# winddori2002/DEX-TTS

Hardware: AMD Instinct MI355X
Metric: mel-frames/s at n_timesteps=50, 80-ch mel (sampler only); RTF (higher is better)
Workload: dtype bf16; 1 GPU; gedex_b1: gedex_lj B=1/GPU T=512 n_timesteps=50 (BASELINE.json configs[1]); global_batch=1, frames=512, hipgraph=False, parallelism=1 GPU

## Files before the change

### dex_tts_amd/csrc/conv3x3_bf16.hip

```cpp
#include "kernels.h"
#include <cstdlib>
#include <cstdio>
#include "lp_util.h"
#include "kernels_lp.h"
#include "conv_gn.h"

namespace dex {
namespace DEX_LP_NS {

typedef float f32x16 __attribute__((ext_vector_type(16)));
typedef unsigned short u16;
typedef unsigned u32x4 __attribute__((ext_vector_type(4)));

__device__ __forceinline__ float cv_mish(float x) {
    const float e = __expf(fminf(x, 20.f));
    const float n = e * (e + 2.f);
    return x * (n * __builtin_amdgcn_rcpf(n + 2.f));
}

template <int NT, int COUT>
__device__ __forceinline__ void cv_epilogue(const Conv3P& p, f32x16 (&acc)[NT], int b, int ho, int w0, int nbase, int lane, int tid,
                                            long long* gnred) {
    const int i = lane & 31, hh = lane >> 5;
    constexpr int cpg = COUT / 8;
// ... 76 lines not shown
    const bool odd = (lane & 1) != 0;
#pragma unroll
    for (int t = 0; t < NT; ++t) {
        const float bias = p.res_b[nb + t * 32 + i];
        if (rfull) {
            float* yp = yl + (odd ? 16 * COUT - 1 : 0) + t * 32;
#pragma unroll
            for (int j = 0; j < 8; ++j) {
                const float lo_r = accr[t][j] + bias, hi_r = accr[t][8 + j] + bias;
                const float recv = lane_xor1(odd ? lo_r : hi_r);
                const float mine = odd ? hi_r : lo_r;
                *reinterpret_cast<float2*>(yp + ((j & 3) + 8 * (j >> 2)) * COUT) = odd ? make_float2(recv, mine) : make_float2(mine, recv);
            }
        } else {
#pragma unroll
            for (int r = 0; r < 16; ++r) {
                const int wo = w0 + (r & 3) + 8 * (r >> 2) + 4 * hh;
                if (ho < p.H && wo < p.W) yl[((r & 3) + 8 * (r >> 2)) * COUT + t * 32] = accr[t][r] + bias;
            }
        }
    }
}

template <int CC, int COUT, int NSL, int TH, bool PRO2 = false, bool RES = false, bool XB = false, int NW = 4, bool RW = false>
__global__ __launch_bounds__(64 * NW) void conv3x3_lp_kernel(const Conv3P p) {
    constexpr int PW = 34, PH = TH + 2;
    constexpr int LDP = CC + 8;
    constexpr int WN = NW / TH;
    constexpr int NTHR = 64 * NW;
    constexpr int NT = NSL / 32 / WN;
    constexpr int NSLICE = COUT / NSL;
    constexpr int ITEMS = PH * PW * (CC / 8);
    constexpr int NI = (ITEMS + NTHR - 1) / NTHR;
    constexpr int WITEMS = NSL * CC / 8;
    constexpr int WPT = (WITEMS + NTHR - 1) / NTHR;
    constexpr bool WFULL = WITEMS % NTHR == 0;
    constexpr int RING = CC == 128 ? (PRO2 ? 1 : 2) : 3;
    constexpr int NPASS = RW ? 1
                        : TH == 5 ? (CC == 128 ? (PRO2 ? 6 : 3) : (PRO2 ? 3 : XB ? 1 : 2))
                                  : CC == 128 ? (TH == 8 ? (PRO2 ? 8 : 4) : (PRO2 ? 5 : 2)) : (PRO2 ? 3 : 1);
    constexpr int NIP = (NI + NPASS - 1) / NPASS;
    constexpr int RWI = 9 * WITEMS;
    constexpr int RWPT = (RWI + NTHR - 1) / NTHR;
    constexpr int RWB = (RWPT + NPASS - 1) / NPASS;
#ifdef DEX_LP_WSPLIT
    constexpr int NTAP = 18;
#else
    constexpr int NTAP = 9;
#endif
    static_assert(NT >= 1 && WPT >= 1 && NW % TH == 0 && NTHR % (CC / 8) == 0, "tile");
    static_assert(!RW || NTAP == 9, "the resident schedule holds nine taps");
    extern __shared__ __attribute__((aligned(16))) u16 smem[];
    u16* patch = smem;
    u16* wbuf = smem + PH * PW * LDP;
    u16* rbuf = wbuf + (RW ? 9 : 2) * NSL * LDP;
    __shared__ long long gnred[16];
    constexpr int COEF_N = (TH == 8) ? 128 : 256;
    __shared__ __attribute__((aligned(16))) float coef[3][COEF_N];

    const int tid = threadIdx.x, lane = tid & 63, wave = tid >> 6;
// ... 44 lines not shown
    if constexpr (RES) {
#pragma unroll
        for (int t = 0; t < NT; ++t)
#pragma unroll
            for (int r = 0; r < 16; ++r) accr[t][r] = 0.f;
    }
    int wofs[WPT], wlds[WPT];
    bool wok[WPT];
#pragma unroll
    for (int j = 0; j < WPT; ++j) {
        const int it = tid + NTHR * j;
        const int n = it / (CC / 8), c8 = (it % (CC / 8)) * 8;
        wofs[j] = n * K + c8;
        wlds[j] = n * LDP + c8;
        wok[j] = WFULL || it < WITEMS;
    }
    const int pc8 = (tid % (CC / 8)) * 8;

    CvGnLoads gnl{};
    if (pro) gnl = cv_gn_issue(p, b, tid, step);
    const int nchunk = RW ? 1 : p.Cin / CC;
    for (int ch = 0; ch < nchunk; ++ch) {
        const int cbase = ch * CC;
        u32x4 w0r[WPT], wr[RING][WPT], rwr[RES ? WPT : 1];
#ifdef DEX_LP_WSPLIT
        u32x4 rwl[RES ? WPT : 1];
#define WS_TAPOFS(t) ((long)((t) % 9) * p.Cin + ((t) >= 9 ? p.w_lo_off : 0L))
#else
#define WS_TAPOFS(t) ((long)(t) * p.Cin)
#endif
        float4 sc0, sc1, sh0, sh1, t0, t1;
#pragma unroll
        for (int ps = 0; ps < NPASS; ++ps) {
            float4 pf0[NIP], pf1[XB ? 1 : NIP], rf0[PRO2 ? NIP : 1], rf1[PRO2 ? NIP : 1];
            float pmk[NIP];
            bool pin[NIP];
#pragma unroll
            for (int q = 0; q < NIP; ++q) {
                const int it = min(tid + NTHR * (ps * NIP + q), ITEMS - 1);
                const int px = it / (CC / 8);
                const int pw = px % PW, ph = px / PW;
                const int hi = h0 + ph - 1, wi = w0 + pw - 1;
                const bool inb = (unsigned)hi < (unsigned)p.H && (unsigned)wi < (unsigned)p.W;
                const int hc = inb ? hi : 0, wc = inb ? wi : 0;
                if constexpr (XB) {
                    pf0[q] = *reinterpret_cast<const float4*>(Xh + ((long)hc * p.W + wc) * p.ldx + cbase + pc8);
                } else {
// ... 87 lines not shown
                    const int px_ = it / (CC / 8), pw_ = px_ % PW, ph_ = px_ / PW;
                    if (slice == 0 && it < ITEMS && pin[q] && ph_ >= 1 && ph_ <= TH && pw_ >= 1 && pw_ <= 32) {
                        float* xo = p.pro_xout + ((long)b * p.H * p.W + (long)(h0 + ph_ - 1) * p.W + (w0 + pw_ - 1)) * p.Cin + cbase + pc8;
                        *reinterpret_cast<float4*>(xo) = f0;
                        *reinterpret_cast<float4*>(xo + 4) = f1;
                    }
                }
                uint4 v;
                v.x = pack2_lp(f0.x * mk, f0.y * mk); v.y = pack2_lp(f0.z * mk, f0.w * mk);
                v.z = pack2_lp(f1.x * mk, f1.y * mk); v.w = pack2_lp(f1.z * mk, f1.w * mk);
                if (it < ITEMS) *reinterpret_cast<uint4*>(patch + (it / (CC / 8)) * LDP + pc8) = v;
            }
            if constexpr (RW) {
#pragma unroll
                for (int j = 0; j < RWB; ++j) {
                    const int it = tid + NTHR * (ps * RWB + j);
                    if (ps * RWB + j < RWPT && (RWI % NTHR == 0 || it < RWI)) {
                        const int r = it % WITEMS;
                        *reinterpret_cast<u32x4*>(wbuf + ((it / WITEMS) * NSL + r / (CC / 8)) * LDP + (r % (CC / 8)) * 8) = rwv[j];
                    }
                }
            }
        }
        if constexpr (!RW) {
#pragma unroll
            for (int j = 0; j < WPT; ++j) if (wok[j]) *reinterpret_cast<u32x4*>(wbuf + wlds[j]) = w0r[j];
        }
        if constexpr (RES) {
#pragma unroll
            for (int j = 0; j < WPT; ++j) if (wok[j]) *reinterpret_cast<u32x4*>(rbuf + wlds[j]) = rwr[j];
        }
        CSTAMP(2);
        if constexpr (RW) {
            lds_barrier();
            constexpr int KS = CC / 16;
            const u16* ap = patch + (wrow * PW + i) * LDP + hh * 8;
            const u16* bp = wbuf + (wcol * NT * 32 + i) * LDP + hh * 8;
            const u16* rp = rbuf + (wcol * NT * 32 + i) * LDP + hh * 8;
            lp8 af[2], bf[2][NT], rf[2][RES ? NT : 1];
            af[0] = *reinterpret_cast<const lp8*>(ap);
#pragma unroll
            for (int t = 0; t < NT; ++t) bf[0][t] = *reinterpret_cast<const lp8*>(bp + t * 32 * LDP);
#pragma unroll
            for (int s = 0; s < 9 * KS; ++s) {
                if (s + 1 < 9 * KS) {
                    const int tap = (s + 1) / KS, ks = (s + 1) % KS, kh = tap / 3, kw = tap - kh * 3;
// ... 6 lines not shown
                            for (int t = 0; t < NT; ++t) rf[(s + 1) & 1][t] = *reinterpret_cast<const lp8*>(rp + t * 32 * LDP + ks * 16);
                        }
                    }
                }
                __builtin_amdgcn_sched_barrier(0);
#pragma unroll
                for (int t = 0; t < NT; ++t) acc[t] = DEX_MFMA_LP(af[s & 1], bf[s & 1][t], acc[t], 0, 0, 0);
                if constexpr (RES) {
                    if (s / KS == 4) {
#pragma unroll
                        for (int t = 0; t < NT; ++t) accr[t] = DEX_MFMA_LP(af[s & 1], rf[s & 1][t], accr[t], 0, 0, 0);
                    }
                }
                __builtin_amdgcn_sched_barrier(0);
            }
        } else {
#pragma unroll
        for (int tt = 0; tt < NTAP; ++tt) {
            const int tap = tt % 9;
            lds_barrier();
            if (tt + 1 < NTAP) {
                u16* wn = wbuf + ((tt + 1) & 1) * NSL * LDP;
#pragma unroll
                for (int j = 0; j < WPT; ++j) if (wok[j]) *reinterpret_cast<u32x4*>(wn + wlds[j]) = wr[tt % RING][j];
                if (tt + 1 + RING < NTAP) {
#pragma unroll
                    for (int j = 0; j < WPT; ++j)
                        if (wok[j]) wr[tt % RING][j] = *reinterpret_cast<const u32x4*>(Wg + wofs[j] + WS_TAPOFS(tt + 1 + RING) + cbase);
                }
                __builtin_amdgcn_sched_barrier(0);
            }
#ifdef DEX_LP_WSPLIT
            if constexpr (RES) {
                if (tt == 5) {
#pragma unroll
                    for (int j = 0; j < WPT; ++j) if (wok[j]) *reinterpret_cast<u32x4*>(rbuf + wlds[j]) = rwl[j];
                }
            }
#endif
            const u16* wb = wbuf + (tt & 1) * NSL * LDP;
            const int kh = tap / 3, kw = tap - kh * 3;
            const u16* ap = patch + ((wrow + kh) * PW + i + kw) * LDP + hh * 8;
            const u16* bp = wb + (wcol * NT * 32 + i) * LDP + hh * 8;
#pragma unroll
            for (int ks = 0; ks < CC / 16; ++ks) {
                const lp8 af = *reinterpret_cast<const lp8*>(ap + ks * 16);
#pragma unroll
                for (int t = 0; t < NT; ++t) {
                    const lp8 bf = *reinterpret_cast<const lp8*>(bp + t * 32 * LDP + ks * 16);
                    acc[t] = DEX_MFMA_LP(af, bf, acc[t], 0, 0, 0);
                }
// ... 7 lines not shown
                    }
                }
            }
        }
        }
    }
    if constexpr (RES) cv_res_store<NT, COUT>(p, accr, b, h0 + wrow, w0, slice * NSL + wcol * NT * 32, lane);
    CSTAMP(3);
    cv_epilogue<NT, COUT>(p, acc, b, h0 + wrow, w0, slice * NSL + wcol * NT * 32, lane, tid, gnred);
#ifdef DEX_TIMING
    CSTAMP(4);
    if (p.dbg && tid == 0) {
        long long* d = p.dbg + ((long)(blockIdx.z * gridDim.y + blockIdx.y) * gridDim.x + blockIdx.x) * 8;
        for (int k = 0; k < 5; ++k) d[k] = tk[k];
        unsigned hw, xcc;
        asm volatile("s_getreg_b32 %0, hwreg(HW_REG_HW_ID)" : "=s"(hw));
        asm volatile("s_getreg_b32 %0, hwreg(HW_REG_XCC_ID)" : "=s"(xcc));
        d[5] = hw; d[6] = xcc & 15u;
        d[7] = __builtin_readcyclecounter() - tk0;
    }
#endif
}

template <int CC, int COUT, int NSL, int TH, bool PRO2 = false, bool RES = false, bool XB = false, int NW = 4, bool RW = false>
static void launch_c3(const Conv3P& p, hipStream_t st) {
    constexpr int LDP = CC + 8;
    const size_t lds = ((size_t)(TH + 2) * 34 * LDP + ((RW ? 9 : 2) + (RES ? 1 : 0)) * NSL * LDP) * sizeof(u16);
    static bool attr = false;
    if (!attr) {
        hipFuncSetAttribute(reinterpret_cast<const void*>(&conv3x3_lp_kernel<CC, COUT, NSL, TH, PRO2, RES, XB, NW, RW>), hipFuncAttributeMaxDynamicSharedMemorySize, (int)lds);
        attr = true;
    }
    dim3 grid((p.W + 31) / 32, (p.H + TH - 1) / TH, p.B * (COUT / NSL));
    if (RW && p.Cin != CC) { fprintf(stderr, "libdexamd: resident conv3x3 form needs Cin == %d in one chunk (got %d)\n", CC, p.Cin); abort(); }
    Conv3P q = p;
    q.skip_dead = (p.B >= 4 && (long)grid.x * grid.y * grid.z >= 1024 && knob_or("DEX_CONV_SKIP_DEAD", 1) != 0) ? 1 : 0;
    static char sym[96];
    if (!sym[0]) snprintf(sym, sizeof sym, "conv3x3_lp_kernel<%d,%d,%d,%d,%d,%d,%d,%d%s>", CC, COUT, NSL, TH, (int)PRO2, (int)RES, (int)XB, NW, RW ? ",resident" : "");
    g_last_symbol = sym;
    hipLaunchKernelGGL((conv3x3_lp_kernel<CC, COUT, NSL, TH, PRO2, RES, XB, NW, RW>), grid, dim3(64 * NW), lds, st, q);
}

bool conv3x3_bf16_tail_supported(int C) {
#if defined(DEX_LP_WSPLIT) && !defined(DEX_WS_HAVE_CONV3)
    return false;
#endif
    return C == 64 || C == 128; }
bool conv3x3_bf16_xb_supported(int Cin, int Cout) {
#if defined(DEX_LP_WSPLIT) && !defined(DEX_WS_HAVE_CONV3)
    return false;
#endif
    return Cin == Cout && (Cin == 64 || Cin == 128); }
bool conv3x3_bf16_res_supported(int Cin, int Cout) {
#if defined(DEX_LP_WSPLIT) && !defined(DEX_WS_HAVE_CONV3_RES)
    return false;
#endif
    return (Cout == 128 && Cin == 64) || (Cout == 64 && (Cin == 128 || Cin == 256)); }
bool conv3x3_bf16_supported(int Cin, int Cout) {
#if defined(DEX_LP_WSPLIT) && !defined(DEX_WS_HAVE_CONV3)
    return false;
#endif
   
    return (Cin == 64 || Cin == 128 || Cin == 256) && (Cout == 64 || Cout == 128);
// ... 137 lines not shown
```

### dex_tts_amd/csrc/dex_api.hip

```cpp
#include <hip/hip_runtime.h>
#include <cstdlib>

#include <cmath>
#include <cstdarg>
#include <atomic>
#include <cstdio>
#include <mutex>
#include <cstring>
#include <map>
#include <unordered_map>
#include <string_view>
#include <string>
#include <vector>

#include "../../include/dex_amd.h"
#include "kernels.h"
#include "weight_store.h"

using namespace dex;

namespace dex {
namespace {
const char* const KNOB_NAMES[] = {
    "DEX_CONV_STREAM", "DEX_CONV_PP", "DEX_CONV_SKIP_DEAD", "DEX_H_BF16", "DEX_ATTN_SEPARATE", "DEX_ATTN_Q64", "DEX_ATTN_Q64_TAIL", "DEX_ATTN_Q64_HALF", "DEX_DIT_XCDS", "DEX_ATTN_GENERIC", "DEX_RES2", "DEX_LP_INTER", "DEX_DIT_CHAIN",
    "DEX_DIT_CLUSTER", "DEX_DIT_CLUSTER_LOCAL", "DEX_ATTN_X_LP", "DEX_RES_X_LP", "DEX_CAT_LP", "DEX_XCD_MAP", "DEX_DEBUG_DROP_HANDOFF", "DEX_PATCH_FUSED",
    "DEX_CONV_DOWN", "DEX_CONVT_UP", "DEX_DEBUG_PLAN",
    "DEX_ATTN_SHARED_W8", "DEX_CONVT_MT", "DEX_CONVT_WGS", "DEX_CONV_DOWN_WGS", "DEX_CONV_REGW", "DEX_CONV_REGW_RES", "DEX_CONV_SMALL_MAX", "DEX_CONV_TH8",
    "DEX_CONV_W8", "DEX_DWCONV_CAP", "DEX_FINAL_CAP", "DEX_FIRST_CAP", "DEX_FIRST_MFMA", "DEX_GEMM_NWALK", "DEX_NWALK_SPLIT", "DEX_NWALK_BM", "DEX_POS_COL", "DEX_POS_COL_MIN",
    "DEX_POS_CT", "DEX_REGW_MIN_TILES", "DEX_REGW_WGS", "DEX_ROWCHAIN64", "DEX_ROWCHAIN64A", "DEX_TIV_CAP", "DEX_TV_CHAIN", "DEX_TIV_FOLD", "DEX_LINATTN_NSUB", "DEX_TV_FOLD", "DEX_OUT2_MIN", "DEX_NWALK_DMA",
    "DEX_LINATTN_HEADWAVES", "DEX_LINATTN_OUT2_HW", "DEX_CONV_ROUND1", "DEX_CONV_RESIDENT", "DEX_KVCTX_ROWS", "DEX_OUT2_ROWS", "DEX_PE_TOK", "DEX_NWALK_SMALL"};
constexpr int N_KNOBS = (int)(sizeof(KNOB_NAMES) / sizeof(KNOB_NAMES[0]));
int knob_parse(const char* e) {
    if (!e) return KNOB_UNSET;
    char* end = nullptr;
    const long v = strtol(e, &end, 10);
    if (end == e) {
        static bool warned = false;
        if (!warned) { warned = true; fprintf(stderr, "libdexamd: ignoring a DEX_* knob whose value '%s' is not an integer\n", e); }
        return KNOB_UNSET;
    }
    return (int)v;
}
struct KnobSnapshot {
    int v[N_KNOBS];
    KnobSnapshot() { for (int i = 0; i < N_KNOBS; ++i) v[i] = knob_parse(getenv(KNOB_NAMES[i])); }
};
thread_local const KnobSnapshot* t_knobs = nullptr;
struct WsplitScope {
    bool prev;
    explicit WsplitScope(bool on) : prev(g_lp_wsplit) { g_lp_wsplit = on; }
    ~WsplitScope() { g_lp_wsplit = prev; }
};
struct KnobScope {
// ... 1888 lines not shown
```

### dex_tts_amd/csrc/dit_rowchain.hip

```cpp
#include <hip/hip_runtime.h>
#include "kernels.h"
#include <cstdlib>
#include "lp_util.h"
#include "kernels_lp.h"

namespace dex {
namespace DEX_LP_NS {

typedef float f32x16 __attribute__((ext_vector_type(16)));
typedef unsigned short u16;

namespace {

constexpr int RC_H = 256, RC_MLP = 512, RC_ROWS = 32, RC_NW = 8;
constexpr int A_LD = RC_H + 8;
constexpr int H_LD = RC_MLP + 8;
constexpr int X_LD = RC_H + 4;
constexpr int AT_LD = 132;
constexpr size_t RC_LDS_ATTN = (size_t)(RC_NW * 32 * AT_LD + RC_NW * 64) * sizeof(float);
constexpr size_t RC_LDS = (size_t)RC_ROWS * (A_LD + H_LD) * sizeof(u16) + (size_t)RC_ROWS * X_LD * sizeof(float) + 4 * RC_H * sizeof(float);

__device__ __forceinline__ float gelu_erf_rc(float x) {
    const float z = fabsf(x) * 0.70710678118654752440f;
    const float t = __builtin_amdgcn_rcpf(fmaf(0.3275911f, z, 1.0f));
// ... 984 lines not shown
    constexpr unsigned SLAB_B = (32 * 256 + 256) * 4;
    const int row = tid >> 4, seg = tid & 15;
    const int nrow = min(n0 + row, N - 1);

#ifdef DEX_TIMING
    long long cts[16] = {0,0,0,0,0,0,0,0,0,0,0,0,0,0,0,0};
    cts[0] = wall_clock64();
#endif
    float4 prm;
    {
        const int which = tid >> 6, c4 = (tid & 63) * 4;
        const float* src = which == 0 ? ada + 3 * RC_H : which == 1 ? ada + 4 * RC_H
                         : which == 2 ? (has_q ? p.next_shift + (long)step * p.next_step_stride : ada)
                         : which == 3 ? (has_q ? p.next_scale + (long)step * p.next_step_stride : ada)
                         : which == 4 ? ada + 2 * RC_H : which == 5 ? (QKV_ONLY ? ada : p.bp) : which == 6 ? ada + 5 * RC_H : (QKV_ONLY ? ada : p.b2);
        prm = *reinterpret_cast<const float4*>(src + c4);
    }
    float4 xr[4];
#pragma unroll
    for (int q = 0; q < 4; ++q) xr[q] = *reinterpret_cast<const float4*>(p.X + (mb + nrow) * RC_H + q * 64 + seg * 4);

    WT8 w8;
    f32x16 acc;
    if constexpr (!QKV_ONLY) {
        const int head = member >> 1, half = member & 1;
        f32x16 ao[4];
        float am = -INFINITY, al = 0.f;
        {
            union DFr { uint4 u; lp8 v; };
            const long hbq = ((long)b * 2 + head) * p.Npad * 16;
            const uint4* Qg = reinterpret_cast<const uint4*>(p.Qin) + hbq + lane;
            const uint4* Kg = reinterpret_cast<const uint4*>(p.Kin) + hbq + lane;
            const uint4* Vg = reinterpret_cast<const uint4*>(p.Vin) + hbq + lane;
            const int ntiles = (N + 31) / 32;
            const int t_lo = half ? (ntiles + 1) / 2 : 0, t_hi = half ? ntiles : (ntiles + 1) / 2;
            DFr qf[8], kf[8], vf[4][2];
            int kt = t_lo + wave;
            {
                const uint4* qp = Qg + (long)(n0 >> 5) * 512;
#pragma unroll
                for (int ks = 0; ks < 8; ++ks) qf[ks].u = qp[ks * 64];
                const long t0 = min(kt, ntiles - 1);
                const uint4* kp = Kg + t0 * 512;
#pragma unroll
                for (int ks = 0; ks < 8; ++ks) kf[ks].u = kp[ks * 64];
                const uint4* vp = Vg + t0 * 512;
// ... 219 lines not shown
    cts[8] = wall_clock64();
#endif
        acc = zero16();
        mma8(acc, w8, Ah + i * CL_AH_LD + hh * 8);
#pragma unroll
        for (int r = 0; r < 16; ++r) P2[((r & 3) + 8 * (r >> 2) + 4 * hh) * X_LD + col] = acc[r];

#ifdef DEX_TIMING
    cts[9] = wall_clock64();
#endif
        lds_barrier();
        {
            const unsigned base = (1 * DIT_CLUSTER + member) * SLAB_B;
#pragma unroll
            for (int q = 0; q < 4; ++q) {
                const float4 v = *reinterpret_cast<const float4*>(P2 + row * X_LD + q * 64 + seg * 4);
                const u32x4v u = {__float_as_uint(v.x), __float_as_uint(v.y), __float_as_uint(v.z), __float_as_uint(v.w)};
                __builtin_amdgcn_raw_buffer_store_b128(u, srs, base + (unsigned)(q * 512 + tid) * 16u, 0, Sc::ST_AUX);
            }
            asm volatile("s_waitcnt vmcnt(0)" ::: "memory");
            __syncthreads();
            if (tid == 0 && !(p.xdrop == 1 && member == 3)) Sc::st(flags + 1 * DIT_CLUSTER + member, flagv);
        }

#ifdef DEX_TIMING
    cts[10] = wall_clock64();
#endif
        cluster_wait<LOCAL>(flags + 1 * DIT_CLUSTER, member, p.epoch, my_xcc, tid, p.xerr);
#ifdef DEX_TIMING
    cts[11] = wall_clock64();
#endif

        {
            u32x4v pv[DIT_CLUSTER][4];
#pragma unroll
            for (int c = 0; c < DIT_CLUSTER; ++c) {
                if (c == member) continue;
                const unsigned base = (1 * DIT_CLUSTER + c) * SLAB_B;
#pragma unroll
                for (int q = 0; q < 4; ++q) pv[c][q] = __builtin_amdgcn_raw_buffer_load_b128(srs, base + (unsigned)(q * 512 + tid) * 16u, 0, Sc::LD_AUX);
            }
#pragma unroll
            for (int q = 0; q < 4; ++q) {
                const float4 own = *reinterpret_cast<const float4*>(P2 + row * X_LD + q * 64 + seg * 4);
                float4 sacc = make_float4(0.f, 0.f, 0.f, 0.f);
#pragma unroll
                for (int c = 0; c < DIT_CLUSTER; ++c) {
                    const float4 pc = c == member ? own : make_float4(__uint_as_float(pv[c][q].x), __uint_as_float(pv[c][q].y), __uint_as_float(pv[c][q].z), __uint_as_float(pv[c][q].w));
                    sacc.x += pc.x; sacc.y += pc.y; sacc.z += pc.z; sacc.w += pc.w;
                }
                const float4 g = *reinterpret_cast<const float4*>(PRM + 6 * RC_H + q * 64 + seg * 4);
                const float4 bb = *reinterpret_cast<const float4*>(PRM + 7 * RC_H + q * 64 + seg * 4);
                const float4 x1 = *reinterpret_cast<const float4*>(X1 + row * X_LD + q * 64 + seg * 4);
                const float4 x2 = make_float4(x1.x + g.x * (sacc.x + bb.x), x1.y + g.y * (sacc.y + bb.y), x1.z + g.z * (sacc.z + bb.z), x1.w + g.w * (sacc.w + bb.w));
                xr[q] = x2;
                if (q == member && n0 + row < N) *reinterpret_cast<float4*>(p.X + (mb + n0 + row) * RC_H + q * 64 + seg * 4) = x2;
            }
        }

#ifdef DEX_TIMING
    cts[12] = wall_clock64();
#endif
        if (!has_q) return;
    } else {
        *reinterpret_cast<float4*>(PRM + (tid >> 6) * RC_H + (tid & 63) * 4) = prm;
        lds_barrier();
    }
    WT16 wq;
    const int nt = 6 * member + wave;
    if (wave < 6) wload(wq, p.Wq, LO_WQ, 16, nt, 0, lane);
    ln_regs_to_A(xr, As, PRM + 2 * RC_H, PRM + 3 * RC_H, row, seg);
    lds_barrier();

#ifdef DEX_TIMING
    cts[13] = wall_clock64();
#endif
    if (wave < 6) {
        acc = zero16();
        if (nt < 16) {
            const QkvBias qb = qkv_bias<0>(p, nt, lane);
            mma16t(acc, wq, As + i * A_LD + hh * 8);
            if (nt < 8) store_qkv_tile_d<0>(p, acc, qb, nt, b, n0, lane); else store_qkv_tile_d<1>(p, acc, qb, nt, b, n0, lane);
        } else {
            const QkvBias qb = qkv_bias<2>(p, nt, lane);
            mma16(acc, wq, As + i * A_LD + hh * 8);
            store_qkv_tile_d<2>(p, acc, qb, nt, b, n0, lane);
        }
    }
#ifdef DEX_TIMING
    cts[14] = wall_clock64();
    if (p.dbg && tid == 0) for (int q = 0; q < 16; ++q) p.dbg[blockIdx.x * 16 + q] = cts[q];
#endif
}
constexpr size_t RC_LDS_CLUSTER_CHAIN = (size_t)(2 * RC_ROWS * X_LD + 8 * RC_H + 4 * RC_ROWS * CL_RED_LD) * sizeof(float)
                                        + (size_t)(RC_ROWS * A_LD + RC_ROWS * CL_AH_LD + RC_NW * RC_ROWS * QK_LD) * sizeof(u16);
constexpr size_t RC_LDS_CLUSTER = RC_LDS_CLUSTER_CHAIN > RC_LDS_ATTN ? RC_LDS_CLUSTER_CHAIN : RC_LDS_ATTN;

bool dit_rowchain_cluster_form(int rows_per_batch, int B) {
#if defined(DEX_LP_WSPLIT) && !defined(DEX_WS_HAVE_RCC)
    return false;
#endif
   
    const int on = knob_or("DEX_DIT_CLUSTER", 1);
    return on && (long)B * ((rows_per_batch + RC_ROWS - 1) / RC_ROWS) * DIT_CLUSTER <= 256;
}

bool dit_rowchain_cluster_local_fits(int rows_per_batch, int B) {
// ... 5 lines not shown
    const long tiles = (long)B * ((rows_per_batch + RC_ROWS - 1) / RC_ROWS);
    const int forced = knob_or("DEX_DIT_XCDS", 0);
    int x = forced >= 1 && forced <= 8 ? forced : 8;
    while (x < 8 && (tiles + x - 1) / x * DIT_CLUSTER > 32) ++x;
    return x;
}

bool dit_rowchain_supported(int hidden, int mlp_hidden) {
#if defined(DEX_LP_WSPLIT) && !defined(DEX_WS_HAVE_RC)
    return false;
#endif
    return hidden == RC_H && mlp_hidden == RC_MLP; }
bool dit_rowchain64_form(int rows_per_batch, int B, int attn_inline) {
#if defined(DEX_LP_WSPLIT) && !defined(DEX_WS_HAVE_RC64)
    return false;
#endif
   
    const int m64 = knob_or("DEX_ROWCHAIN64", 1);
    const long wg32 = (long)B * ((rows_per_batch + RC_ROWS - 1) / RC_ROWS);
    const bool small_n = dit_sep64_small_n(rows_per_batch, B);
    return m64 && !attn_inline && (m64 == 2 || wg32 >= 768 || small_n);
}

void launch_dit_rowchain(const DitChainP& p, hipStream_t st) {
    if (p.xslab && (p.attn_inline || p.qkv_only) && dit_rowchain_cluster_form(p.rows_per_batch, p.B)) {
        static bool attrc = false;
        if (!attrc) {
            hipFuncSetAttribute(reinterpret_cast<const void*>(&dit_rowchain_cluster_kernel<false, false>), hipFuncAttributeMaxDynamicSharedMemorySize, (int)RC_LDS_CLUSTER);
            hipFuncSetAttribute(reinterpret_cast<const void*>(&dit_rowchain_cluster_kernel<false, true>), hipFuncAttributeMaxDynamicSharedMemorySize, (int)RC_LDS_CLUSTER);
            hipFuncSetAttribute(reinterpret_cast<const void*>(&dit_rowchain_cluster_kernel<true, false>), hipFuncAttributeMaxDynamicSharedMemorySize, (int)RC_LDS_CLUSTER);
            attrc = true;
        }
        const int tiles = p.B * ((p.rows_per_batch + RC_ROWS - 1) / RC_ROWS);
        const int xc = p.xlocal ? (p.xcds >= 1 && p.xcds <= 8 ? p.xcds : 8) : 8;
        const dim3 gridc((p.xlocal ? (tiles + xc - 1) / xc * 8 : tiles) * DIT_CLUSTER);
        if (p.qkv_only) {
            g_last_symbol = "dit_rowchain_cluster_kernel<true,false>";
            hipLaunchKernelGGL((dit_rowchain_cluster_kernel<true, false>), gridc, dim3(RC_NW * 64), RC_LDS_CLUSTER, st, p);
        } else if (p.xdrop == 2) {
            DitChainP q = p; q.xlocal = 0;
            g_last_symbol = "dit_rowchain_cluster_kernel<false,true>";
            hipLaunchKernelGGL((dit_rowchain_cluster_kernel<false, true>), dim3(tiles * DIT_CLUSTER), dim3(RC_NW * 64), RC_LDS_CLUSTER, st, q);
        } else if (p.xlocal) {
            g_last_symbol = "dit_rowchain_cluster_kernel<false,true>";
            hipLaunchKernelGGL((dit_rowchain_cluster_kernel<false, true>), gridc, dim3(RC_NW * 64), RC_LDS_CLUSTER, st, p);
        } else {
            g_last_symbol = "dit_rowchain_cluster_kernel<false,false>";
// ... 78 lines not shown
```

### dex_tts_amd/csrc/kernels.h

```cpp
#pragma once
#include <hip/hip_runtime.h>
#include <stdint.h>

namespace dex {

constexpr int KNOB_UNSET = -2147483647 - 1;
int knob(const char* name);
inline int knob_or(const char* name, int dflt) { const int v = knob(name); return v == KNOB_UNSET ? dflt : v; }
inline bool knob_off(const char* name) { return knob(name) == 0; }
inline bool knob_set(const char* name) { return knob(name) != KNOB_UNSET; }
inline int device_cus() {
    static const int n = [] { int dev = 0, v = 0; (void)hipGetDevice(&dev); (void)hipDeviceGetAttribute(&v, hipDeviceAttributeMultiprocessorCount, dev); return v > 0 ? v : 256; }();
    return n;
}

constexpr int GN_SLOTS = 32;
typedef long long gnfix_t;

extern thread_local const char* g_last_symbol;

constexpr int PREC_FP32 = 0, PREC_BF16 = 1, PREC_FP16 = 2, PREC_FP16X2 = 3;
inline bool prec_wsplit(int precision) { return precision == PREC_FP16X2; }
extern thread_local bool g_lp_wsplit;
inline bool prec_is_lp(int precision) { return precision != PREC_FP32; }
// ... 190 lines not shown
void launch_pos_finish(const PosFinishP& p, hipStream_t st);
void launch_group_pad(const float* src, float* dst, long rows, int G, int cg, int cg_pad, hipStream_t st);

struct LnModP { const float* X; float* Y; int rows_per_batch; int D; const float* shift; const float* scale;
                long step_stride; int step; int B; int row_bstride = 0; };
void launch_ln_mod(const LnModP& p, hipStream_t st);

struct DitChainP { const float* O; int ksplit; long o_sstride; const float* ml; int heads; int rows_per_batch;
                   float* X; const void *Wp, *W1, *W2, *Wq; const float *bp, *b1, *b2, *bq;
                   const float* ada;
                   const float *next_shift, *next_scale; long next_step_stride;
                   void *Qh, *Kh, *Vt; int Npad; float qscale;
                   const void *Qin, *Kin, *Vin;
                   int qkv_only;
                   int attn_inline;
                   int step; int M; int B; long long* dbg;
                   float* xslab; unsigned* xflag; unsigned epoch; int* xerr;
                   int o_lp;
                   int xcd_map;
                   int xlocal;
                   int xdrop;
                   int tail_row0 = 0, tail_ks = 0;
                   int row_bstride = 0;
                   int xcds = 8; };
constexpr int DIT_CLUSTER = 4;
constexpr size_t DIT_CLUSTER_SLAB_FLOATS = 2 * DIT_CLUSTER * (32 * 256 + 256);
constexpr size_t DIT_CLUSTER_FLAG_WORDS = 2 * DIT_CLUSTER;
bool dit_rowchain64_form(int rows_per_batch, int B, int attn_inline);
bool dit_rowchain_cluster_form(int rows_per_batch, int B);
bool dit_rowchain_cluster_local_fits(int rows_per_batch, int B);
int dit_rowchain_cluster_xcds(int rows_per_batch, int B);
bool dit_rowchain_supported(int hidden, int mlp_hidden);
struct AttnDirectP { const void *Qh, *Kh, *Vt; int N, Npad, B; float* O; long o_sstride; float* ml; int ksplit; long long* dbg;
                     int o_lp;
                     int xcd_map;
                     int tail_g = 0, tail_ks = 0;
                     int half_g = 0, half_n = 0; };
void launch_attention_direct(const AttnDirectP& p, int precision, hipStream_t st);
bool attention_direct_batch_regime(int N, int B);
int attention_direct_ksplit(int N, int B);
void launch_attention_q64(const AttnDirectP& p, int precision, hipStream_t st);
int attention_q64_ksplit(int N, int B, int max_split);
void attention_q64_plan(int N, int B, int max_split, int* ks, int* tail_g, int* tail_ks);
bool attention_q64_half_plan(int N, int B, int* half_g, int* half_n);
void launch_dit_rowchain(const DitChainP& p, int precision, hipStream_t st);
void launch_pack_lp_frag(const float* src, void* dst, int K, int N, int precision, hipStream_t st);
void launch_pack_lp_frag_nk(const float* src, void* dst, int K, int N, int precision, hipStream_t st);
// ... 139 lines not shown
```

### dex_tts_amd/csrc/linattn_fused.hip

```cpp
#include "kernels.h"
#include "lp_util.h"
#include "kernels_lp.h"

namespace dex {
namespace DEX_LP_NS {

typedef float f32x16 __attribute__((ext_vector_type(16)));
typedef unsigned short u16;
union LFrag { uint4 u; lp8 v; };
constexpr float LOG2E_F = 1.4426950408889634f;


#ifdef DEX_TIMING
#define KSTAMP_DECL long long tk[8] = {0, 0, 0, 0, 0, 0, 0, 0}; const long long tk0 = __builtin_readcyclecounter(); long long tlast = tk0;
#define KSTAMP(k) do { const long long now_ = __builtin_readcyclecounter(); tk[k] += now_ - tlast; tlast = now_; } while (0)
#define KSTAMP_STORE(n)                                                                                               \
    if (p.dbg && threadIdx.x == 0) {                                                                                  \
        long long* d_ = p.dbg + ((long)blockIdx.y * gridDim.x + blockIdx.x) * 8;                                      \
        for (int k_ = 0; k_ < (n); ++k_) d_[k_] = tk[k_];                                                             \
        d_[7] = __builtin_readcyclecounter() - tk0;                                                                   \
    }
#else
#define KSTAMP_DECL
#define KSTAMP(k) do {} while (0)
// ... 798 lines not shown
            bia[g4] = *reinterpret_cast<const float4*>(p.bias + co);
        }
#pragma unroll
        for (int ks = 0; ks < 8; ++ks) {
            LFrag af; af.u = w2f[ct][ks];
            y = DEX_MFMA_LP(af.v, qf[ks].v, y, 0, 0, 0);
        }
        KSTAMP(4);
        if (ok) {
#pragma unroll
            for (int g4 = 0; g4 < 4; ++g4) {
                const int co = ct * 32 + 8 * g4 + 4 * hh;
                float4 o;
                o.x = y[g4 * 4 + 0] + res[g4].x + bia[g4].x; o.y = y[g4 * 4 + 1] + res[g4].y + bia[g4].y;
                o.z = y[g4 * 4 + 2] + res[g4].z + bia[g4].z; o.w = y[g4 * 4 + 3] + res[g4].w + bia[g4].w;
                *reinterpret_cast<float4*>(Y + (long)(px0 + i) * p.ldy + co) = o;
            }
        }
        KSTAMP(5);
    }
    KSTAMP_STORE(7)
}

template <int C, bool ROWS = false>
__global__ __launch_bounds__(256) void linattn_out2_hw_kernel(const LinOut2P p) {
    constexpr int KS1 = C / 16, CT = C / 32, KQ = KS1 / 4;
    constexpr int O8 = C / 8, XH = ROWS ? 33 : 32, LDY = C + 4;
    __shared__ uint4 xs[KS1][2 * XH], qs[8][64];
    __shared__ __attribute__((aligned(16))) float ys[ROWS ? 32 * LDY : 4];
    KSTAMP_DECL
    const int tid = threadIdx.x, lane = tid & 63;
    const int t = __builtin_amdgcn_readfirstlane(tid >> 6);
    const int i = lane & 31, hh = lane >> 5;
    const int fi = hh * XH + i;
    const int b = blockIdx.y;
    const int px0 = blockIdx.x * 32;
    if (px0 >= p.npix) return;
    const float* X = p.X + (long)b * p.xb + p.x_coff;
    const int px = min(px0 + i, p.npix - 1);
    const int rp0 = 8 * t + lane / O8, rch = 8 * (lane % O8);
    float4 xa[KQ], xc[KQ];
    if constexpr (ROWS) {
#pragma unroll
        for (int k = 0; k < KQ; ++k) {
            const float* xr = X + (long)min(px0 + rp0 + k * (64 / O8), p.npix - 1) * p.ldx + rch;
            xa[k] = *reinterpret_cast<const float4*>(xr);
            xc[k] = *reinterpret_cast<const float4*>(xr + 4);
        }
    } else {
        const float* xr = X + (long)px * p.ldx + hh * 8;
#pragma unroll
        for (int k = 0; k < KQ; ++k) {
            const int ks = t * KQ + k;
            xa[k] = *reinterpret_cast<const float4*>(xr + ks * 16);
            xc[k] = *reinterpret_cast<const float4*>(xr + ks * 16 + 4);
        }
    }
    const uint4* wq = reinterpret_cast<const uint4*>(p.Wq) + lane;
    uint4 wqf[KS1];
#ifdef DEX_LP_WSPLIT
    uint4 wql[KS1];
#endif
#pragma unroll
    for (int ks = 0; ks < KS1; ++ks) {
        wqf[ks] = wq[(t * KS1 + ks) * 64];
// ... 12 lines not shown
    }
    if constexpr (ROWS) {
        bia[0] = *reinterpret_cast<const float4*>(p.bias + rch);
        bia[1] = *reinterpret_cast<const float4*>(p.bias + rch + 4);
    } else if (g2) {
        if constexpr (C != 128) {
#pragma unroll
            for (int g4 = 0; g4 < 4; ++g4) res[g4] = *reinterpret_cast<const float4*>(X + (long)px * p.ldx + ct * 32 + 8 * g4 + 4 * hh);
        }
        const float4* bt = reinterpret_cast<const float4*>(p.bias + ct * 32);
        const unsigned hm = 0u - (unsigned)hh;
#pragma unroll
        for (int g4 = 0; g4 < 4; ++g4) {
            const float4 b0 = bt[2 * g4], b1 = bt[2 * g4 + 1];
            bia[g4] = make_float4(__uint_as_float((__float_as_uint(b1.x) & hm) | (__float_as_uint(b0.x) & ~hm)),
                                  __uint_as_float((__float_as_uint(b1.y) & hm) | (__float_as_uint(b0.y) & ~hm)),
                                  __uint_as_float((__float_as_uint(b1.z) & hm) | (__float_as_uint(b0.z) & ~hm)),
                                  __uint_as_float((__float_as_uint(b1.w) & hm) | (__float_as_uint(b0.w) & ~hm)));
        }
    }
    KSTAMP(0);
#pragma unroll
    for (int k = 0; k < KQ; ++k) {
        LFrag f;
        f.u.x = pack2_lp(xa[k].x, xa[k].y); f.u.y = pack2_lp(xa[k].z, xa[k].w);
        f.u.z = pack2_lp(xc[k].x, xc[k].y); f.u.w = pack2_lp(xc[k].z, xc[k].w);
        if constexpr (ROWS) xs[rch >> 4][((rch >> 3) & 1) * XH + rp0 + k * (64 / O8)] = f.u;
        else xs[t * KQ + k][fi] = f.u;
    }
    if constexpr (C == 128 && !ROWS) {
#pragma unroll
        for (int k = 0; k < 2; ++k) {
            const float4 snd = hh ? xa[k] : xc[k];
            float4 rcv;
            rcv.x = __shfl_xor(snd.x, 32); rcv.y = __shfl_xor(snd.y, 32); rcv.z = __shfl_xor(snd.z, 32); rcv.w = __shfl_xor(snd.w, 32);
            res[2 * k] = hh ? rcv : xa[k];
            res[2 * k + 1] = hh ? xc[k] : rcv;
        }
    }
    lds_barrier();
    KSTAMP(1);
    {
        f32x16 q;
#pragma unroll
        for (int r = 0; r < 16; ++r) q[r] = 0.f;
#pragma unroll
// ... 24 lines not shown
#pragma unroll
        for (int ks = 0; ks < 8; ++ks) {
            LFrag af, qf; af.u = w2f[ks]; qf.u = qs[ks][lane];
            y = DEX_MFMA_LP(af.v, qf.v, y, 0, 0, 0);
        }
    }
    KSTAMP(4);
    float* Y = p.Y + (long)b * p.yb + p.y_coff;
    if constexpr (ROWS) {
        if (g2) {
#pragma unroll
            for (int g4 = 0; g4 < 4; ++g4)
                *reinterpret_cast<float4*>(ys + i * LDY + ct * 32 + 8 * g4 + 4 * hh) = make_float4(y[g4 * 4 + 0], y[g4 * 4 + 1], y[g4 * 4 + 2], y[g4 * 4 + 3]);
        }
        lds_barrier();
#pragma unroll
        for (int k = 0; k < KQ; ++k) {
            const int rp = rp0 + k * (64 / O8);
            const float4 ya = *reinterpret_cast<const float4*>(ys + rp * LDY + rch), yc = *reinterpret_cast<const float4*>(ys + rp * LDY + rch + 4);
            if (px0 + rp < p.npix) {
                float4 oa, oc;
                oa.x = ya.x + xa[k].x + bia[0].x; oa.y = ya.y + xa[k].y + bia[0].y; oa.z = ya.z + xa[k].z + bia[0].z; oa.w = ya.w + xa[k].w + bia[0].w;
                oc.x = yc.x + xc[k].x + bia[1].x; oc.y = yc.y + xc[k].y + bia[1].y; oc.z = yc.z + xc[k].z + bia[1].z; oc.w = yc.w + xc[k].w + bia[1].w;
                float* yr = Y + (long)(px0 + rp) * p.ldy + rch;
                *reinterpret_cast<float4*>(yr) = oa;
                *reinterpret_cast<float4*>(yr + 4) = oc;
            }
        }
    } else if (px0 + i < p.npix) {
#pragma unroll
        for (int g4 = 0; g4 < 4; ++g4) {
            const int co = ct * 32 + 8 * g4 + 4 * hh;
            float4 o;
            o.x = y[g4 * 4 + 0] + res[g4].x + bia[g4].x; o.y = y[g4 * 4 + 1] + res[g4].y + bia[g4].y;
            o.z = y[g4 * 4 + 2] + res[g4].z + bia[g4].z; o.w = y[g4 * 4 + 3] + res[g4].w + bia[g4].w;
            *reinterpret_cast<float4*>(Y + (long)(px0 + i) * p.ldy + co) = o;
        }
    }
    KSTAMP(5);
    KSTAMP_STORE(7)
}
template <int C>
__global__ __launch_bounds__(256) __attribute__((amdgpu_waves_per_eu(2, C == 64 ? 4 : 2))) void linattn_out2_kernel(const LinOut2P p) {
    constexpr int KS1 = C / 16, CT = C / 32;
    constexpr int LDX = C + 4;
    constexpr int NCH = 32 * C / 4 / 64;
    extern __shared__ __attribute__((aligned(16))) float smem_o2[];
    const int tid = threadIdx.x, lane = tid & 63, wave = tid >> 6;
    const int i = lane & 31, hh = lane >> 5;
// ... 107 lines not shown
                u16* y2 = reinterpret_cast<u16*>(p.Y2) + (long)b * p.y2b + p.y2_coff + (long)(px0 + px) * p.ldy2 + ch;
                *reinterpret_cast<uint2*>(y2) = make_uint2(pack2_lp(o.x, o.y), pack2_lp(o.z, o.w));
            }
        }
    }
}
bool linattn_fused_supported(int C) {
#if defined(DEX_LP_WSPLIT) && !defined(DEX_WS_HAVE_LINATTN)
    return false;
#endif
    return C == 64 || C == 128;
}
static long out2_min_wgs() { return knob_or("DEX_OUT2_MIN", 256); }
bool linattn_out2_lp_out_supported(int npix, int B) { return (long)((npix + 127) / 128) * B >= out2_min_wgs(); }
void launch_linattn_out2(const LinOut2P& p, hipStream_t st) {
    dim3 grid((p.npix + 127) / 128, p.B);
    const size_t lds = (size_t)4 * 32 * (p.C + 4) * sizeof(float);
    static bool attr = false;
    if (!attr) {
        hipFuncSetAttribute(reinterpret_cast<const void*>(&linattn_out2_kernel<128>), hipFuncAttributeMaxDynamicSharedMemorySize, (int)((size_t)4 * 32 * 132 * sizeof(float)));
        attr = true;
    }
    const bool lp_io = p.x_lp || p.y_lp || p.Y2;
    if (p.hw && !lp_io) {
        g_last_symbol = "linattn_out2_hw_kernel";
        const dim3 g1((p.npix + 31) / 32, p.B);
        if (p.rows) {
            if (p.C == 64) hipLaunchKernelGGL((linattn_out2_hw_kernel<64, true>), g1, dim3(256), 0, st, p);
            else hipLaunchKernelGGL((linattn_out2_hw_kernel<128, true>), g1, dim3(256), 0, st, p);
            return;
        }
        if (p.C == 64) hipLaunchKernelGGL((linattn_out2_hw_kernel<64, false>), g1, dim3(256), 0, st, p);
        else hipLaunchKernelGGL((linattn_out2_hw_kernel<128, false>), g1, dim3(256), 0, st, p);
        return;
    }
    if ((long)grid.x * p.B < out2_min_wgs()) {
        if (p.C == 64) hipLaunchKernelGGL(linattn_out2_direct_kernel<64>, grid, dim3(256), 0, st, p);
        else hipLaunchKernelGGL(linattn_out2_direct_kernel<128>, grid, dim3(256), 0, st, p);
        return;
    }
    if (p.C == 64) hipLaunchKernelGGL(linattn_out2_kernel<64>, grid, dim3(256), lds, st, p);
    else hipLaunchKernelGGL(linattn_out2_kernel<128>, grid, dim3(256), lds, st, p);
}

}
}
// ... 1 lines not shown
```

Measured before the change: 29820 mel-frames/s.

## Add deeper conv weight ring, early DiT Wq load, and bf16-IO out2 hw kernel

Three separate changes. The conv3x3 kernel gets an optional deeper weight-prefetch ring behind DEX_CONV_RING_LATE (off by default), and the DiT rowchain kernel can issue its Wq weight and bias loads earlier behind DEX_DIT_WQ_EARLY (off by default). The linattn_out2 head-wave kernel gains a 16-bit row-IO variant that reads and writes bf16 activations directly. That variant is on by default for C=64 with aligned strides, replacing the direct or LDS kernel on that path. The deeper ring and early loads raise register pressure, and the bf16 path adds unpack and pack work to save memory traffic.

```diff
diff --git a/dex_tts_amd/csrc/conv3x3_bf16.hip b/dex_tts_amd/csrc/conv3x3_bf16.hip
--- a/dex_tts_amd/csrc/conv3x3_bf16.hip
+++ b/dex_tts_amd/csrc/conv3x3_bf16.hip
@@ -122,7 +122,7 @@
     }
 }
 
-template <int CC, int COUT, int NSL, int TH, bool PRO2 = false, bool RES = false, bool XB = false, int NW = 4, bool RW = false>
+template <int CC, int COUT, int NSL, int TH, bool PRO2 = false, bool RES = false, bool XB = false, int NW = 4, bool RW = false, int RL = 0>
 __global__ __launch_bounds__(64 * NW) void conv3x3_lp_kernel(const Conv3P p) {
     constexpr int PW = 34, PH = TH + 2;
     constexpr int LDP = CC + 8;
@@ -136,6 +136,8 @@
     constexpr int WPT = (WITEMS + NTHR - 1) / NTHR;
     constexpr bool WFULL = WITEMS % NTHR == 0;
     constexpr int RING = CC == 128 ? (PRO2 ? 1 : 2) : 3;
+    constexpr int RINGL = RL > RING ? RL : RING;
+    static_assert(RL == 0 || (!RW && RL > RING), "a late ring is deeper than the entry ring, streamed forms only");
     constexpr int NPASS = RW ? 1
                         : TH == 5 ? (CC == 128 ? (PRO2 ? 6 : 3) : (PRO2 ? 3 : XB ? 1 : 2))
                                   : CC == 128 ? (TH == 8 ? (PRO2 ? 8 : 4) : (PRO2 ? 5 : 2)) : (PRO2 ? 3 : 1);
@@ -226,7 +228,7 @@
     const int nchunk = RW ? 1 : p.Cin / CC;
     for (int ch = 0; ch < nchunk; ++ch) {
         const int cbase = ch * CC;
-        u32x4 w0r[WPT], wr[RING][WPT], rwr[RES ? WPT : 1];
+        u32x4 w0r[WPT], wr[RINGL][WPT], rwr[RES ? WPT : 1];
 #ifdef DEX_LP_WSPLIT
         u32x4 rwl[RES ? WPT : 1];
 #define WS_TAPOFS(t) ((long)((t) % 9) * p.Cin + ((t) >= 9 ? p.w_lo_off : 0L))
@@ -360,6 +362,16 @@
                 }
             }
         }
+        if constexpr (RINGL > RING) {
+#pragma unroll
+            for (int s = RING; s < RINGL; ++s) {
+                if (s + 1 < NTAP) {
+#pragma unroll
+                    for (int j = 0; j < WPT; ++j) if (wok[j]) wr[s][j] = *reinterpret_cast<const u32x4*>(Wg + wofs[j] + WS_TAPOFS(s + 1) + cbase);
+                }
+            }
+            __builtin_amdgcn_sched_barrier(0);
+        }
         if constexpr (!RW) {
 #pragma unroll
             for (int j = 0; j < WPT; ++j) if (wok[j]) *reinterpret_cast<u32x4*>(wbuf + wlds[j]) = w0r[j];
@@ -412,11 +424,11 @@
             if (tt + 1 < NTAP) {
                 u16* wn = wbuf + ((tt + 1) & 1) * NSL * LDP;
 #pragma unroll
-                for (int j = 0; j < WPT; ++j) if (wok[j]) *reinterpret_cast<u32x4*>(wn + wlds[j]) = wr[tt % RING][j];
-                if (tt + 1 + RING < NTAP) {
+                for (int j = 0; j < WPT; ++j) if (wok[j]) *reinterpret_cast<u32x4*>(wn + wlds[j]) = wr[tt % RINGL][j];
+                if (tt + 1 + RINGL < NTAP) {
 #pragma unroll
                     for (int j = 0; j < WPT; ++j)
-                        if (wok[j]) wr[tt % RING][j] = *reinterpret_cast<const u32x4*>(Wg + wofs[j] + WS_TAPOFS(tt + 1 + RING) + cbase);
+                        if (wok[j]) wr[tt % RINGL][j] = *reinterpret_cast<const u32x4*>(Wg + wofs[j] + WS_TAPOFS(tt + 1 + RINGL) + cbase);
                 }
                 __builtin_amdgcn_sched_barrier(0);
             }
@@ -470,13 +482,20 @@
 #endif
 }
 
-template <int CC, int COUT, int NSL, int TH, bool PRO2 = false, bool RES = false, bool XB = false, int NW = 4, bool RW = false>
+constexpr int c3_ring_late(bool pro2, bool res, bool xb) { return 4; }
+
+template <int CC, int COUT, int NSL, int TH, bool PRO2 = false, bool RES = false, bool XB = false, int NW = 4, bool RW = false, int RL = 0>
 static void launch_c3(const Conv3P& p, hipStream_t st) {
+#ifndef DEX_LP_WSPLIT
+    if constexpr (RL == 0 && CC == 128 && NSL == 64 && TH == 2 && NW == 4 && !RW) {
+        if (knob_or("DEX_CONV_RING_LATE", 0) != 0) { launch_c3<CC, COUT, NSL, TH, PRO2, RES, XB, NW, RW, c3_ring_late(PRO2, RES, XB)>(p, st); return; }
+    }
+#endif
     constexpr int LDP = CC + 8;
     const size_t lds = ((size_t)(TH + 2) * 34 * LDP + ((RW ? 9 : 2) + (RES ? 1 : 0)) * NSL * LDP) * sizeof(u16);
     static bool attr = false;
     if (!attr) {
-        hipFuncSetAttribute(reinterpret_cast<const void*>(&conv3x3_lp_kernel<CC, COUT, NSL, TH, PRO2, RES, XB, NW, RW>), hipFuncAttributeMaxDynamicSharedMemorySize, (int)lds);
+        hipFuncSetAttribute(reinterpret_cast<const void*>(&conv3x3_lp_kernel<CC, COUT, NSL, TH, PRO2, RES, XB, NW, RW, RL>), hipFuncAttributeMaxDynamicSharedMemorySize, (int)lds);
         attr = true;
     }
     dim3 grid((p.W + 31) / 32, (p.H + TH - 1) / TH, p.B * (COUT / NSL));
@@ -486,7 +505,7 @@
     static char sym[96];
     if (!sym[0]) snprintf(sym, sizeof sym, "conv3x3_lp_kernel<%d,%d,%d,%d,%d,%d,%d,%d%s>", CC, COUT, NSL, TH, (int)PRO2, (int)RES, (int)XB, NW, RW ? ",resident" : "");
     g_last_symbol = sym;
-    hipLaunchKernelGGL((conv3x3_lp_kernel<CC, COUT, NSL, TH, PRO2, RES, XB, NW, RW>), grid, dim3(64 * NW), lds, st, q);
+    hipLaunchKernelGGL((conv3x3_lp_kernel<CC, COUT, NSL, TH, PRO2, RES, XB, NW, RW, RL>), grid, dim3(64 * NW), lds, st, q);
 }
 
 bool conv3x3_bf16_tail_supported(int C) {
diff --git a/dex_tts_amd/csrc/dex_api.hip b/dex_tts_amd/csrc/dex_api.hip
--- a/dex_tts_amd/csrc/dex_api.hip
+++ b/dex_tts_amd/csrc/dex_api.hip
@@ -28,7 +28,8 @@
     "DEX_ATTN_SHARED_W8", "DEX_CONVT_MT", "DEX_CONVT_WGS", "DEX_CONV_DOWN_WGS", "DEX_CONV_REGW", "DEX_CONV_REGW_RES", "DEX_CONV_SMALL_MAX", "DEX_CONV_TH8",
     "DEX_CONV_W8", "DEX_DWCONV_CAP", "DEX_FINAL_CAP", "DEX_FIRST_CAP", "DEX_FIRST_MFMA", "DEX_GEMM_NWALK", "DEX_NWALK_SPLIT", "DEX_NWALK_BM", "DEX_POS_COL", "DEX_POS_COL_MIN",
     "DEX_POS_CT", "DEX_REGW_MIN_TILES", "DEX_REGW_WGS", "DEX_ROWCHAIN64", "DEX_ROWCHAIN64A", "DEX_TIV_CAP", "DEX_TV_CHAIN", "DEX_TIV_FOLD", "DEX_LINATTN_NSUB", "DEX_TV_FOLD", "DEX_OUT2_MIN", "DEX_NWALK_DMA",
-    "DEX_LINATTN_HEADWAVES", "DEX_LINATTN_OUT2_HW", "DEX_CONV_ROUND1", "DEX_CONV_RESIDENT", "DEX_KVCTX_ROWS", "DEX_OUT2_ROWS", "DEX_PE_TOK", "DEX_NWALK_SMALL"};
+    "DEX_LINATTN_HEADWAVES", "DEX_LINATTN_OUT2_HW", "DEX_CONV_ROUND1", "DEX_CONV_RESIDENT", "DEX_KVCTX_ROWS", "DEX_OUT2_ROWS", "DEX_PE_TOK", "DEX_NWALK_SMALL",
+    "DEX_DIT_WQ_EARLY", "DEX_OUT2_HW16", "DEX_OUT2_HW16_CAP", "DEX_CONV_RING_LATE"};
 constexpr int N_KNOBS = (int)(sizeof(KNOB_NAMES) / sizeof(KNOB_NAMES[0]));
 int knob_parse(const char* e) {
     if (!e) return KNOB_UNSET;
diff --git a/dex_tts_amd/csrc/dit_rowchain.hip b/dex_tts_amd/csrc/dit_rowchain.hip
--- a/dex_tts_amd/csrc/dit_rowchain.hip
+++ b/dex_tts_amd/csrc/dit_rowchain.hip
@@ -1030,6 +1030,10 @@
 
     WT8 w8;
     f32x16 acc;
+    WT16 wq;
+    QkvBias qb;
+    const int nt = 6 * member + wave;
+    const bool wq_early = !QKV_ONLY && has_q && p.wq_early != 0;
     if constexpr (!QKV_ONLY) {
         const int head = member >> 1, half = member & 1;
         f32x16 ao[4];
@@ -1295,6 +1299,10 @@
             __syncthreads();
             if (tid == 0 && !(p.xdrop == 1 && member == 3)) Sc::st(flags + 1 * DIT_CLUSTER + member, flagv);
         }
+        if (wq_early && wave < 6) {
+            wload(wq, p.Wq, LO_WQ, 16, nt, 0, lane);
+            qb = nt < 16 ? qkv_bias<0>(p, nt, lane) : qkv_bias<2>(p, nt, lane);
+        }
 
 #ifdef DEX_TIMING
     cts[10] = wall_clock64();
@@ -1339,9 +1347,7 @@
         *reinterpret_cast<float4*>(PRM + (tid >> 6) * RC_H + (tid & 63) * 4) = prm;
         lds_barrier();
     }
-    WT16 wq;
-    const int nt = 6 * member + wave;
-    if (wave < 6) wload(wq, p.Wq, LO_WQ, 16, nt, 0, lane);
+    if (!wq_early && wave < 6) wload(wq, p.Wq, LO_WQ, 16, nt, 0, lane);
     ln_regs_to_A(xr, As, PRM + 2 * RC_H, PRM + 3 * RC_H, row, seg);
     lds_barrier();
 
@@ -1351,11 +1357,11 @@
     if (wave < 6) {
         acc = zero16();
         if (nt < 16) {
-            const QkvBias qb = qkv_bias<0>(p, nt, lane);
+            if (!wq_early) qb = qkv_bias<0>(p, nt, lane);
             mma16t(acc, wq, As + i * A_LD + hh * 8);
             if (nt < 8) store_qkv_tile_d<0>(p, acc, qb, nt, b, n0, lane); else store_qkv_tile_d<1>(p, acc, qb, nt, b, n0, lane);
         } else {
-            const QkvBias qb = qkv_bias<2>(p, nt, lane);
+            if (!wq_early) qb = qkv_bias<2>(p, nt, lane);
             mma16(acc, wq, As + i * A_LD + hh * 8);
             store_qkv_tile_d<2>(p, acc, qb, nt, b, n0, lane);
         }
@@ -1407,7 +1413,9 @@
     return m64 && !attn_inline && (m64 == 2 || wg32 >= 768 || small_n);
 }
 
-void launch_dit_rowchain(const DitChainP& p, hipStream_t st) {
+void launch_dit_rowchain(const DitChainP& p0, hipStream_t st) {
+    DitChainP p = p0;
+    p.wq_early = knob_or("DEX_DIT_WQ_EARLY", 0) != 0 ? 1 : 0;
     if (p.xslab && (p.attn_inline || p.qkv_only) && dit_rowchain_cluster_form(p.rows_per_batch, p.B)) {
         static bool attrc = false;
         if (!attrc) {
diff --git a/dex_tts_amd/csrc/kernels.h b/dex_tts_amd/csrc/kernels.h
--- a/dex_tts_amd/csrc/kernels.h
+++ b/dex_tts_amd/csrc/kernels.h
@@ -236,7 +236,8 @@
                    int xdrop;
                    int tail_row0 = 0, tail_ks = 0;
                    int row_bstride = 0;
-                   int xcds = 8; };
+                   int xcds = 8;
+                   int wq_early = 0; };
 constexpr int DIT_CLUSTER = 4;
 constexpr size_t DIT_CLUSTER_SLAB_FLOATS = 2 * DIT_CLUSTER * (32 * 256 + 256);
 constexpr size_t DIT_CLUSTER_FLAG_WORDS = 2 * DIT_CLUSTER;
diff --git a/dex_tts_amd/csrc/linattn_fused.hip b/dex_tts_amd/csrc/linattn_fused.hip
--- a/dex_tts_amd/csrc/linattn_fused.hip
+++ b/dex_tts_amd/csrc/linattn_fused.hip
@@ -844,8 +844,9 @@
     KSTAMP_STORE(7)
 }
 
-template <int C, bool ROWS = false>
+template <int C, bool ROWS = false, bool LP16 = false>
 __global__ __launch_bounds__(256) void linattn_out2_hw_kernel(const LinOut2P p) {
+    static_assert(ROWS || !LP16, "16-bit rows exist in the ROWS form only");
     constexpr int KS1 = C / 16, CT = C / 32, KQ = KS1 / 4;
     constexpr int O8 = C / 8, XH = ROWS ? 33 : 32, LDY = C + 4;
     __shared__ uint4 xs[KS1][2 * XH], qs[8][64];
@@ -862,7 +863,13 @@
     const int px = min(px0 + i, p.npix - 1);
     const int rp0 = 8 * t + lane / O8, rch = 8 * (lane % O8);
     float4 xa[KQ], xc[KQ];
-    if constexpr (ROWS) {
+    const bool xlp = LP16 && p.x_lp != 0;
+    if (xlp) {
+        const u16* Xh = reinterpret_cast<const u16*>(p.X) + (long)b * p.xb + p.x_coff;
+#pragma unroll
+        for (int k = 0; k < KQ; ++k)
+            xa[k] = *reinterpret_cast<const float4*>(Xh + (long)min(px0 + rp0 + k * (64 / O8), p.npix - 1) * p.ldx + rch);
+    } else if constexpr (ROWS) {
 #pragma unroll
         for (int k = 0; k < KQ; ++k) {
             const float* xr = X + (long)min(px0 + rp0 + k * (64 / O8), p.npix - 1) * p.ldx + rch;
@@ -921,6 +928,11 @@
     KSTAMP(0);
 #pragma unroll
     for (int k = 0; k < KQ; ++k) {
+        if (xlp) {
+            const unsigned u0 = __float_as_uint(xa[k].x), u1 = __float_as_uint(xa[k].y), u2 = __float_as_uint(xa[k].z), u3 = __float_as_uint(xa[k].w);
+            xa[k] = make_float4(lp_lo(u0), lp_hi(u0), lp_lo(u1), lp_hi(u1));
+            xc[k] = make_float4(lp_lo(u2), lp_hi(u2), lp_lo(u3), lp_hi(u3));
+        }
         LFrag f;
         f.u.x = pack2_lp(xa[k].x, xa[k].y); f.u.y = pack2_lp(xa[k].z, xa[k].w);
         f.u.z = pack2_lp(xc[k].x, xc[k].y); f.u.w = pack2_lp(xc[k].z, xc[k].w);
@@ -991,9 +1003,18 @@
                 float4 oa, oc;
                 oa.x = ya.x + xa[k].x + bia[0].x; oa.y = ya.y + xa[k].y + bia[0].y; oa.z = ya.z + xa[k].z + bia[0].z; oa.w = ya.w + xa[k].w + bia[0].w;
                 oc.x = yc.x + xc[k].x + bia[1].x; oc.y = yc.y + xc[k].y + bia[1].y; oc.z = yc.z + xc[k].z + bia[1].z; oc.w = yc.w + xc[k].w + bia[1].w;
-                float* yr = Y + (long)(px0 + rp) * p.ldy + rch;
-                *reinterpret_cast<float4*>(yr) = oa;
-                *reinterpret_cast<float4*>(yr + 4) = oc;
+                if (LP16 && p.y_lp) {
+                    u16* yh = reinterpret_cast<u16*>(p.Y) + (long)b * p.yb + p.y_coff + (long)(px0 + rp) * p.ldy + rch;
+                    *reinterpret_cast<uint4*>(yh) = make_uint4(pack2_lp(oa.x, oa.y), pack2_lp(oa.z, oa.w), pack2_lp(oc.x, oc.y), pack2_lp(oc.z, oc.w));
+                } else {
+                    float* yr = Y + (long)(px0 + rp) * p.ldy + rch;
+                    *reinterpret_cast<float4*>(yr) = oa;
+                    *reinterpret_cast<float4*>(yr + 4) = oc;
+                }
+                if (LP16 && p.Y2) {
+                    u16* y2 = reinterpret_cast<u16*>(p.Y2) + (long)b * p.y2b + p.y2_coff + (long)(px0 + rp) * p.ldy2 + rch;
+                    *reinterpret_cast<uint4*>(y2) = make_uint4(pack2_lp(oa.x, oa.y), pack2_lp(oa.z, oa.w), pack2_lp(oc.x, oc.y), pack2_lp(oc.z, oc.w));
+                }
             }
         }
     } else if (px0 + i < p.npix) {
@@ -1147,6 +1168,16 @@
         attr = true;
     }
     const bool lp_io = p.x_lp || p.y_lp || p.Y2;
+    if (lp_io && p.C == 64 && p.rows && knob_or("DEX_OUT2_HW16", 1) != 0 && !knob_off("DEX_LINATTN_OUT2_HW")) {
+        const long g128 = (long)grid.x * p.B;
+        const bool al = (!p.x_lp || (p.ldx % 8 == 0 && p.x_coff % 8 == 0 && p.xb % 8 == 0)) && (!p.y_lp || (p.ldy % 8 == 0 && p.y_coff % 8 == 0 && p.yb % 8 == 0))
+                        && (!p.Y2 || (p.ldy2 % 8 == 0 && p.y2_coff % 8 == 0 && p.y2b % 8 == 0));
+        if (al && (long)grid.x >= out2_min_wgs() && g128 <= knob_or("DEX_OUT2_HW16_CAP", 320)) {
+            g_last_symbol = "linattn_out2_hw_kernel<64,rows,lp16>";
+            hipLaunchKernelGGL((linattn_out2_hw_kernel<64, true, true>), dim3((p.npix + 31) / 32, p.B), dim3(256), 0, st, p);
+            return;
+        }
+    }
     if (p.hw && !lp_io) {
         g_last_symbol = "linattn_out2_hw_kernel";
         const dim3 g1((p.npix + 31) / 32, p.B);
```

Result: no change. 29860 mel-frames/s, median of 3 (+0.2%).
